# DonghuiZhuo/kube-batch-1

Measured on AMD Instinct MI355X. Metric: pod placements/sec + p50 session latency, 100k nodes × 1M pods, higher is better.
Workload: dtype int64

## Files before the change

kube-batch-1_amd/csrc/engine/engine_placer.h:

```cpp
#pragma once
#include <hip/hip_runtime.h>

#define KBHIP_STAMPS_OFF
#include "../kbhip_batch.h"
#include "../kbhip_engine.h"
#include "engine_dev.h"

namespace kbhip {

static_assert(sizeof(Row) == 4 * (kPkFlags - kPkRow), "the package carries a Row as 28 32-bit words");
static_assert(kEngDescClass + sizeof(TaskClass) / 4 <= kEngDescWords, "a descriptor carries its class");

template <typename ET>
__device__ __forceinline__ Row eng_row_after(const TaskClass& c, const PlaceDec<ET>& D, const Row& base) {
    const int cc = D.cc > 0 ? D.cc : 0;
    const int na = cc < D.ap_l ? cc : D.ap_l;
    return apply_commits(base, c, na, cc - na);
}
template <typename ET>
__device__ __forceinline__ void eng_fit_vals(const Conf& cf, const NodeCols& nc, const DevTables& t,
                                             const TaskClass& c, const PopArgs& a, const PlaceDec<ET>& D,
                                             const Row& base, const int32_t* fit_in, uint32_t fit_raw, uint64_t* g0,
                                             uint64_t* g1) {
    uint32_t fb_base = 0, fb_post = 0;
// ... 191 lines not shown
                                             const TaskClass& c, int node, const Row& r) {
    const uint64_t pw[4] = {0, 0, 0, 0};
    int32_t sc;
    bool passed;
    const int32_t na = cf.score_mult ? na_weight(c, t, nc, node) : 0;
    const uint64_t k1 = dyn_key(cf, c, t, nc, apply_commits(r, c, 1, 0), pw, node, true, na, &sc, &passed);
    return k1 ? key_score(k1) : INT32_MIN;
}
__device__ __forceinline__ bool front_wait(const EngPlacerLds& L, const int* seq, int want) {
    while (__hip_atomic_load(seq, __ATOMIC_RELAXED, __HIP_MEMORY_SCOPE_WORKGROUP) != want) {
        if (!__hip_atomic_load(&L.ok, __ATOMIC_RELAXED, __HIP_MEMORY_SCOPE_WORKGROUP)) return false;
        __builtin_amdgcn_s_sleep(1);
    }
    return true;
}

template <bool LIST>
__device__ __forceinline__ void eng_front_eval(const Conf& cf, const NodeCols& nc, const DevTables& t,
                                               const EngArgs& A, EngPlacerLds& L, uint32_t q, uint32_t dw, int set,
                                               int role) {
    const int lane = eng_lane();
    uint32_t w[8];
#pragma unroll
    for (int i = 0; i < 8; ++i) w[i] = (uint32_t)__builtin_amdgcn_readlane((int)dw, i);
    const EngDesc d = eng_decode(w);
    const PopArgs a = eng_args(d);
    const TaskClass c = eng_class_x(dw);
    const int ring = (int)((q + 3 - set) % 4);
    const int sl = 64 * ring + lane;
    if (!LIST && set == 0) {
        if (!front_wait(L, &L.rows_seq, (int)(q - 1))) return;
        const int node = L.xn[ring][lane];
        if (role == 0) {
            ETL(A, q - 1, 32);
            FrontKey k{0u, 0u, 0u, 0, INT32_MIN};
            if (node >= 0) k = front_key(cf, nc, t, c, a, node, L.rc.row[sl], L.flags[sl]);
            ETL(A, q - 1, 33);
            L.fe[0][lane] = k.e;
            L.ffb[0][lane] = (uint8_t)k.fb;
            L.fkind[0][lane] = (uint8_t)k.kind;
            L.fna[0][lane] = k.na;
            if (k.kind == 2) L.fs1p[0][lane] = k.s1p;
            ETL(A, q - 1, 34);
            L.e[0][lane] = wave_sort_desc(node >= 0 ? k.e : 0u);
            L.fbp[0][lane] = node >= 0 ? (uint8_t)k.fb : (uint8_t)0;
            __builtin_amdgcn_s_waitcnt(0xc07f);
            if (lane == 0) __hip_atomic_store(&L.sort_seq[0], (int)q, __ATOMIC_RELAXED, __HIP_MEMORY_SCOPE_WORKGROUP);
            ETL(A, q - 1, 35);
        } else if (node >= 0) {
            L.fs1a[0][lane] = front_s1a(cf, nc, t, c, node, L.rc.row[sl]);
        }
        return;
    }
    if (set == 0) {
        if (!front_wait(L, &L.xn_seq, (int)(q - 1))) return;
        const int node = L.xn[ring][lane];
        const int src = node >= 0 ? L.srcslot[lane] : 0;
        const bool own_ring = src >= 64 * ring && src < 64 * ring + 64;
        if (role == 0) {
            FrontKey k{0u, 0u, 0u, 0, INT32_MIN};
            if (node >= 0) k = front_key(cf, nc, t, c, a, node, L.rc.row[src], L.flags[src]);
            if (!front_wait(L, &L.rows_seq, (int)(q - 1))) return;
            ETL(A, q - 1, 32);
            const int m = L.ccm[lane];
            if (m == 1 && node >= 0 && !own_ring) {
                if (!front_wait(L, &L.v1_seq[0], (int)q)) return;
                k.e = L.v1e[lane]; k.fb = L.v1fb[lane]; k.kind = L.v1kind[lane]; k.s1p = L.v1s1p[lane];
            }
            const bool slow = node >= 0 && (m > 1 || own_ring);
            if (__ballot(slow) != 0 && slow) k = front_key(cf, nc, t, c, a, node, L.rc.row[sl], L.flags[sl]);
            ETL(A, q - 1, 33);
            L.fe[0][lane] = k.e;
            L.ffb[0][lane] = (uint8_t)k.fb;
            L.fkind[0][lane] = (uint8_t)k.kind;
            L.fna[0][lane] = k.na;
            if (k.kind == 2) L.fs1p[0][lane] = k.s1p;
            ETL(A, q - 1, 34);
            L.e[0][lane] = wave_sort_desc(node >= 0 ? k.e : 0u);
            L.fbp[0][lane] = node >= 0 ? (uint8_t)k.fb : (uint8_t)0;
            __builtin_amdgcn_s_waitcnt(0xc07f);
            if (lane == 0) __hip_atomic_store(&L.sort_seq[0], (int)q, __ATOMIC_RELAXED, __HIP_MEMORY_SCOPE_WORKGROUP);
            ETL(A, q - 1, 35);
        } else {
            int32_t s1 = INT32_MIN;
            if (node >= 0) s1 = front_s1a(cf, nc, t, c, node, L.rc.row[src]);
            if (!front_wait(L, &L.rows_seq, (int)(q - 1))) return;
            const int m = L.ccm[lane];
            if (m == 1 && node >= 0 && !own_ring) {
                if (!front_wait(L, &L.v1_seq[1], (int)q)) return;
                s1 = L.v1s1a[lane];
            }
            const bool slow = node >= 0 && (m > 1 || own_ring);
            if (__ballot(slow) != 0 && slow) s1 = front_s1a(cf, nc, t, c, node, L.rc.row[sl]);
            if (node >= 0) L.fs1a[0][lane] = s1;
        }
        return;
    }
    if (role == 0) ETL(A, q - 1, 32 + 4 * set);
    const int node = L.xn[ring][lane];
    if (role == 0) {
        FrontKey k{0u, 0u, 0u, 0, INT32_MIN};
        if (node >= 0) k = front_key(cf, nc, t, c, a, node, L.rc.row[sl], L.flags[sl]);
        ETL(A, q - 1, 33 + 4 * set);
        L.fe[set][lane] = k.e;
        L.ffb[set][lane] = (uint8_t)k.fb;
        L.fkind[set][lane] = (uint8_t)k.kind;
        L.fna[set][lane] = k.na;
        if (k.kind == 2) L.fs1p[set][lane] = k.s1p;
        bool hashed = false;
        for (int i = 0; i < 4096 && !hashed; ++i) {
            hashed = __hip_atomic_load(&L.hash_seq, __ATOMIC_RELAXED, __HIP_MEMORY_SCOPE_WORKGROUP) == (int)q;
            if (!hashed) __builtin_amdgcn_s_sleep(1);
        }
        ETL(A, q - 1, 34 + 4 * set);
        if (hashed) {
            const bool use = node >= 0 && (set == 1 ? L.x2use[lane] : L.x3use[lane]);
            L.e[set][lane] = wave_sort_desc(use ? k.e : 0u);
            L.fbp[set][lane] = use ? (uint8_t)k.fb : (uint8_t)0;
            __builtin_amdgcn_s_waitcnt(0xc07f);
            if (lane == 0) __hip_atomic_store(&L.sort_seq[set], (int)q, __ATOMIC_RELAXED, __HIP_MEMORY_SCOPE_WORKGROUP);
            ETL(A, q - 1, 35 + 4 * set);
        }
    } else if (node >= 0) {
        L.fs1a[set][lane] = front_s1a(cf, nc, t, c, node, L.rc.row[sl]);
    }
}

__device__ __forceinline__ void eng_front_v1(const Conf& cf, const NodeCols& nc, const DevTables& t,
                                             EngPlacerLds& L, uint32_t q, uint32_t dw, int role) {
    const int lane = eng_lane();
    uint32_t w[8];
#pragma unroll
    for (int i = 0; i < 8; ++i) w[i] = (uint32_t)__builtin_amdgcn_readlane((int)dw, i);
    const PopArgs a = eng_args(eng_decode(w));
    const TaskClass c = eng_class_x(dw);
    if (!front_wait(L, &L.xn_seq, (int)(q - 1))) return;
    const TaskClass& cp = *(const TaskClass*)&L.desc[(q - 1) % 2][kEngDescClass];
    const int ring = (int)((q + 3) % 4);
    const int node = L.xn[ring][lane];
    if (node >= 0) {
        const int src = L.srcslot[lane];
        const Row r = apply_commits(L.rc.row[src], cp, 1, 0);
        if (role == 0) {
            const FrontKey k = front_key(cf, nc, t, c, a, node, r, L.flags[src]);
            L.v1e[lane] = k.e; L.v1fb[lane] = (uint8_t)k.fb; L.v1kind[lane] = (uint8_t)k.kind; L.v1s1p[lane] = k.s1p;
        } else {
            L.v1s1a[lane] = front_s1a(cf, nc, t, c, node, r);
        }
    }
    __builtin_amdgcn_s_waitcnt(0xc07f);
    if (lane == 0) __hip_atomic_store(&L.v1_seq[role], (int)q, __ATOMIC_RELAXED, __HIP_MEMORY_SCOPE_WORKGROUP);
}

template <int K>
__device__ __forceinline__ void front_pkg_store(EngPlacerLds& L, const uint64_t (&v)[16], int base, uint32_t q,
                                                int lane) {
    EngRowCache& rc = L.rc;
#pragma unroll
    for (int i = 0; i < 16; ++i) {
        constexpr int kF0 = 8 * K;
        const int f = kF0 + (i >> 1), e = lane + 64 * (i & 1), sl = base + e;
        const uint32_t x = (uint32_t)v[i];
        if (f == kPkKey) L.pkey[q % 2][e] = x;
        else if (f < kPkFlags) ((uint32_t*)&rc.row[sl])[f - kPkRow] = x;
        else if (f == kPkFlags) L.flags[sl] = (uint8_t)x;
        else if (f == kPkNa) rc.na[sl] = (int32_t)x;
        else rc.s1[sl] = (int32_t)x;
    }
}

template <bool LIST>
__device__ __forceinline__ void eng_front(const Conf& cf, const NodeCols& nc, const DevTables& t, const EngArgs& A,
                                          EngPlacerLds& L, uint32_t q, int wave) {
    const int lane = threadIdx.x & 63;
    EngCtl* ctl = A.ctl;
    EngRowCache& rc = L.rc;
    if (wave == 0) return;
    const int k = wave == 3 ? 0 : wave == 4 ? 1 : wave - 4;
    const EngPkg* pk = A.pkg + (q % kEngSlots);
    uint64_t v[16];
    uint32_t dw;
    if (__hip_atomic_load(&L.ndesc_seq, __ATOMIC_RELAXED, __HIP_MEMORY_SCOPE_WORKGROUP) == (int)q) {
        dw = L.ndesc[lane];
    } else {
        const uint64_t* src = &ctl->desc[q % kEngRing][lane];
        EngWait wt(ctl, kEngDescTicks);
        uint64_t x = 0;
        for (;;) {
            x = ld_sc1(src);
            if (__ballot((uint32_t)(x >> 32) != q) == 0) break;
            if (!wt.tick(kEngErrDesc)) {
                if (wave == 3 && lane == 0) L.ok = 0;
                return;
            }
        }
        dw = (uint32_t)x;
    }
    if (wave == 3) L.desc[q % 2][lane] = dw;
    if (((uint32_t)__builtin_amdgcn_readlane((int)dw, kDwFlags) >> 12 & 0xf) != kEngOpPop) return;
    if (wave == 2) {
        const int r1 = (int)((q + 3) % 4), r2 = (int)((q + 2) % 4), r3 = (int)((q + 1) % 4);
        while (__hip_atomic_load(&L.xn_seq, __ATOMIC_RELAXED, __HIP_MEMORY_SCOPE_WORKGROUP) != (int)(q - 1)) {
            if (!__hip_atomic_load(&L.ok, __ATOMIC_RELAXED, __HIP_MEMORY_SCOPE_WORKGROUP)) return;
            __builtin_amdgcn_s_sleep(1);
        }
        for (int h = lane; h < EngRowCache::kHashN; h += 64) rc.hkey[h] = -1;
        __builtin_amdgcn_s_waitcnt(0xc07f);
        __builtin_amdgcn_wave_barrier();
        const int n1 = L.xn[r1][lane];
        if (n1 >= 0) rc_insert(&rc, n1, 64 * r1 + lane);
        __builtin_amdgcn_s_waitcnt(0xc07f);
        __builtin_amdgcn_wave_barrier();
        const int n2 = L.xn[r2][lane];
        const bool use2 = n2 >= 0 && rc_find(&rc, n2) < 0;
        L.x2use[lane] = use2;
        if (use2) rc_insert(&rc, n2, 64 * r2 + lane);
        if (!LIST) {
            __builtin_amdgcn_s_waitcnt(0xc07f);
            __builtin_amdgcn_wave_barrier();
            const int n3 = L.xn[r3][lane];
            const bool use3 = n3 >= 0 && rc_find(&rc, n3) < 0;
            L.x3use[lane] = use3;
            if (use3) rc_insert(&rc, n3, 64 * r3 + lane);
        }
        __builtin_amdgcn_s_waitcnt(0xc07f);
        if (lane == 0) __hip_atomic_store(&L.hash_seq, (int)q, __ATOMIC_RELAXED, __HIP_MEMORY_SCOPE_WORKGROUP);
        ETL(A, q - 1, 63);
        eng_front_eval<LIST>(cf, nc, t, A, L, q, dw, 0, 1);
        return;
    }
    if constexpr (LIST) {
        if (wave == 1) { eng_front_eval<LIST>(cf, nc, t, A, L, q, dw, 0, 0); return; }
        if (wave == 5) { eng_front_v1(cf, nc, t, L, q, dw, 1); return; }
        if (wave == 3) eng_front_eval<LIST>(cf, nc, t, A, L, q, dw, 1, 1);
        else if (wave == 6) eng_front_eval<LIST>(cf, nc, t, A, L, q, dw, 1, 0);
        else if (wave == 7) eng_front_v1(cf, nc, t, L, q, dw, 0);
    } else {
        if (wave == 1) { eng_front_eval<LIST>(cf, nc, t, A, L, q, dw, 0, 0); return; }
        if (wave == 5) { eng_front_eval<LIST>(cf, nc, t, A, L, q, dw, 1, 1); return; }
        if (wave == 3) eng_front_eval<LIST>(cf, nc, t, A, L, q, dw, 2, 1);
        else if (wave == 6) eng_front_eval<LIST>(cf, nc, t, A, L, q, dw, 1, 0);
        else if (wave == 7) eng_front_eval<LIST>(cf, nc, t, A, L, q, dw, 2, 0);
    }
    ETL(A, q - 1, 56 + k);
    bool got = false;
    if (!eng_poll_tag(ctl, &ctl->pkg_ready[q % kEngSlots][0], q, kEngWaitTicks)) {
        if (k == 0 && lane == 0) L.ok = 0;
        return;
    }
#pragma unroll
    for (int i = 0; i < 16; ++i) v[i] = ld_sc1(&pk->w[8 * k + (i >> 1)][lane + 64 * (i & 1)]);
    EngWait wt(ctl, kEngWaitTicks);
    for (;;) {
        bool miss = false;
#pragma unroll
        for (int i = 0; i < 16; ++i) miss |= (uint32_t)(v[i] >> 32) != q;
        if (__ballot(miss) == 0) { got = true; break; }
#pragma unroll
        for (int i = 0; i < 16; ++i)
            if ((uint32_t)(v[i] >> 32) != q) v[i] = ld_sc1(&pk->w[8 * k + (i >> 1)][lane + 64 * (i & 1)]);
        if (!wt.tick()) break;
    }
    if (got) {
        ETL(A, q - 1, 48 + k);
        const int base = kEngStage + kEngPkgN * (int)(q % 2);
        switch (k) {
            case 0: front_pkg_store<0>(L, v, base, q, lane); break;
            case 1: front_pkg_store<1>(L, v, base, q, lane); break;
            case 2: front_pkg_store<2>(L, v, base, q, lane); break;
            default: front_pkg_store<3>(L, v, base, q, lane); break;
        }
        ETL(A, q - 1, 52 + k);
        if (k == 0) {
            for (int w = 0; w < 4; ++w) { rc.pw[base + lane][w] = 0; rc.pw[base + 64 + lane][w] = 0; }
            bool hashed = false;
            for (int i = 0; i < 4096 && !hashed; ++i) {
                hashed = __hip_atomic_load(&L.hash_seq, __ATOMIC_RELAXED, __HIP_MEMORY_SCOPE_WORKGROUP) == (int)q;
                if (!hashed) __builtin_amdgcn_s_sleep(1);
            }
            ETL(A, q - 1, 62);
            if (hashed) {
                uint32_t w8[8];
#pragma unroll
                for (int i = 0; i < 8; ++i) w8[i] = (uint32_t)__builtin_amdgcn_readlane((int)dw, i);
                eng_drop_stale(L, eng_args(eng_decode(w8)), q);
                __builtin_amdgcn_s_waitcnt(0xc07f);
                if (lane == 0) __hip_atomic_store(&L.drop_seq, (int)q, __ATOMIC_RELAXED, __HIP_MEMORY_SCOPE_WORKGROUP);
                ETL(A, q - 1, 60);
                bool both = false;
                for (int i = 0; i < 4096 && !both; ++i) {
                    both = __hip_atomic_load(&L.sort_seq[1], __ATOMIC_RELAXED, __HIP_MEMORY_SCOPE_WORKGROUP) == (int)q &&
                           (LIST ||
                            __hip_atomic_load(&L.sort_seq[2], __ATOMIC_RELAXED, __HIP_MEMORY_SCOPE_WORKGROUP) == (int)q);
                    if (!both) __builtin_amdgcn_s_sleep(1);
                }
                if (both) {
                    uint32_t top = wave_merge_desc(L.s64[lane], L.e[1][lane]);
                    L.pre64[lane] = LIST ? top : wave_merge_desc(top, L.e[2][lane]);
                    __builtin_amdgcn_s_waitcnt(0xc07f);
                    if (lane == 0) __hip_atomic_store(&L.pre_seq, (int)q, __ATOMIC_RELAXED, __HIP_MEMORY_SCOPE_WORKGROUP);
                    ETL(A, q - 1, 61);
                }
            }
        }
    } else if (k == 0 && lane == 0) {
        L.ok = 0;
    }
}

template <bool LIST>
__device__ __forceinline__ void eng_placer(const Conf& cf, const NodeCols& nc, const DevTables& t, const EngArgs& A,
                                           EngPlacerLds& L) {
    const int lane = threadIdx.x & 63, wave = threadIdx.x >> 6;
    EngCtl* ctl = A.ctl;
    EngRowCache& rc = L.rc;
    for (int i = threadIdx.x; i < 4 * 64; i += kPopThreads) L.xn[i >> 6][i & 63] = -1;
    if (threadIdx.x == 0) {
        L.ok = 1; L.gran_seq = 0; L.ndesc_seq = 0; L.rows_seq = (int)A.first - 1;
        L.hash_seq = L.drop_seq = (int)A.first - 1;
        L.xn_seq = (int)A.first - 1;
        L.v1_seq[0] = L.v1_seq[1] = L.pre_seq = (int)A.first - 1;
        L.sort_seq[0] = L.sort_seq[1] = L.sort_seq[2] = (int)A.first - 1;
        L.apmin = A.first - 1;
    }
    __syncthreads();
    eng_front<LIST>(cf, nc, t, A, L, A.first, wave);
    uint32_t pend = 0;
    for (uint32_t p = A.first;; ++p) {
        const int r1 = (int)((p + 3) % 4), r2 = (int)((p + 2) % 4), r3 = (int)((p + 1) % 4), r0 = (int)(p % 4);
        __syncthreads();
        if (!L.ok) return;
        const EngDesc d = eng_decode(L.desc[p % 2]);
        if (d.op != kEngOpPop) {
            if (wave == 0) eng_publish_done(ctl, &pend);
            return;
        }
        const PopArgs a = eng_args(d);
        const TaskClass& c = *(const TaskClass*)&L.desc[p % 2][kEngDescClass];
        if (wave == 0) {
            ETL(A, p, 0);
            if (lane == 0 && A.tl) A.tl[(size_t)(p % kEngTlSlots) * kEngTlEvents + 31] = p;
        }
        if (wave == 0) {
            if (__hip_atomic_load(&L.drop_seq, __ATOMIC_RELAXED, __HIP_MEMORY_SCOPE_WORKGROUP) != (int)p)
                eng_drop_stale(L, a, p);
            ETL(A, p, 1);
        } else if (wave == 4) {
            const uint64_t x = ld_sc1(&ctl->desc[(p + 1) % kEngRing][lane]);
            if (__ballot((uint32_t)(x >> 32) != p + 1) == 0) {
                L.ndesc[lane] = (uint32_t)x;
                __builtin_amdgcn_s_waitcnt(0xc07f);
                if (lane == 0) __hip_atomic_store(&L.ndesc_seq, (int)(p + 1), __ATOMIC_RELAXED, __HIP_MEMORY_SCOPE_WORKGROUP);
            }
        } else if (wave == 1 || wave == 5 || (!LIST && wave == 6)) {
            const int set = wave == 1 ? 0 : wave - 4;
            const int ring = set == 0 ? r1 : set == 1 ? r2 : r3;
            const int node = L.xn[ring][lane];
            const bool use = node >= 0 && (set == 0 || (set == 1 ? L.x2use[lane] : L.x3use[lane]));
            if (wave == 1) ETL(A, p, 2);
            if (__hip_atomic_load(&L.sort_seq[set], __ATOMIC_RELAXED, __HIP_MEMORY_SCOPE_WORKGROUP) != (int)p) {
                L.e[set][lane] = wave_sort_desc(use ? L.fe[set][lane] : 0u);
                L.fbp[set][lane] = use ? L.ffb[set][lane] : (uint8_t)0;
            }
            if (wave == 1) ETL(A, p, 9);
            if (use) {
                const int sl = 64 * ring + lane;
                const int kind = L.fkind[set][lane];
                rc.na[sl] = L.fna[set][lane];
                rc.s1[sl] = kind == 0 ? INT32_MIN : kind == 2 ? L.fs1p[set][lane] : L.fs1a[set][lane];
            }
        }
        __syncthreads();
        if (wave == 0) ETL(A, p, 3);
        if (wave == 0) {
            uint32_t top;
            if (__hip_atomic_load(&L.pre_seq, __ATOMIC_RELAXED, __HIP_MEMORY_SCOPE_WORKGROUP) == (int)p) {
                top = wave_merge_desc(L.pre64[lane], L.e[0][lane]);
            } else {
                top = wave_merge_desc(L.s64[lane], L.e[0][lane]);
                top = wave_merge_desc(top, L.e[1][lane]);
                if (!LIST) top = wave_merge_desc(top, L.e[2][lane]);
            }
            const uint32_t fbp = (uint32_t)L.fbp[0][lane] | ((uint32_t)L.fbp[1][lane] << 4) |
                                 (LIST ? 0u : ((uint32_t)L.fbp[2][lane] << 8));
#pragma unroll
            for (int q = 0; q < 4; ++q) {
                const int k = __popcll(__ballot((fbp >> q) & 1u)) + __popcll(__ballot((fbp >> (q + 4)) & 1u)) +
                              __popcll(__ballot((fbp >> (q + 8)) & 1u));
                if (lane == q) L.fitin[q] = k;
            }
            const int n = top ? key_node(top, a) : -1;
            ETL(A, p, 44);
            eng_publish_done(ctl, &pend);
            ETL(A, p, 45);
            if constexpr (LIST) {
                if ((int32_t)(L.apmin - (p - kEngLog)) < 0 && !eng_own_apmin(A, L, p - kEngLog)) {
                    if (lane == 0) __hip_atomic_store(&L.ok, 0, __ATOMIC_RELAXED, __HIP_MEMORY_SCOPE_WORKGROUP);
                }
                st_sc1(&ctl->tlog[p % kEngLog][lane], ((uint64_t)p << 32) | (uint32_t)n);
                if (lane == 0) st_sc1(&ctl->tcls[p % kEngLog], ((uint64_t)p << 32) | (uint32_t)a.cls);
            } else {
#pragma unroll
                for (int cp = 0; cp < kEngCandCopies; ++cp)
                    st_sc1(&ctl->cands[p % kEngSlots][cp][lane], ((uint64_t)p << 32) | (uint32_t)n);
            }
            ETL(A, p, 46);
            int src = n >= 0 ? rc_find(&rc, n) : -1;
            if (n >= 0 && src < 0) {
                src = 64 * r0 + lane;
                const Row r = load_row_sc1(nc, n);
                const int32_t na = cf.score_mult ? na_weight(c, t, nc, n) : 0;
                const uint64_t pw[4] = {0, 0, 0, 0};
                rc.row[src] = r;
                L.flags[src] = nc.flags[n];
                rc.na[src] = na;
                rc.s1[src] = depth1_score(cf, nc, t, c, r, pw, n, na, key64_of(top, a));
                for (int w = 0; w < 4; ++w) rc.pw[src][w] = 0;
            }
            L.srcslot[lane] = src;
            L.xn[r0][lane] = n;
            L.wl64[0][lane] = key64_of(top, a);
            __builtin_amdgcn_s_waitcnt(0xc07f);
            if (lane == 0) __hip_atomic_store(&L.xn_seq, (int)p, __ATOMIC_RELAXED, __HIP_MEMORY_SCOPE_WORKGROUP);
            ETL(A, p, 4);
            ETL(A, p, 5);
        }
        if (wave == 0) {
            PlaceDec<uint32_t> D;
            if (place_decide_wave<uint32_t, true>(cf, nc, t, c, a, L.wl64[0], p, &rc, L.srcslot, !A.quick, D)) {
                ETL(A, p, 6);
                if (lane == 0 && A.tl)
                    A.tl[(size_t)(p % kEngTlSlots) * kEngTlEvents + 30] = (uint64_t)D.done | ((uint64_t)D.stop << 8);
                eng_finish<LIST>(cf, nc, t, c, a, A, L, p, r0, D, &pend);
            } else if (lane == 0) {
                __hip_atomic_store(&ctl->err, (uint32_t)kEngErrClass, __ATOMIC_RELAXED, __HIP_MEMORY_SCOPE_AGENT);
                __hip_atomic_store(&L.ok, 0, __ATOMIC_RELAXED, __HIP_MEMORY_SCOPE_WORKGROUP);
            }
        } else {
            if (wave == 5) eng_host_out(A, L, p, d.slot);
            eng_front<LIST>(cf, nc, t, A, L, p + 1, wave);
            if (wave == 3) ETL(A, p, 15);
            if (wave == 1) ETL(A, p, 19);
            if (wave == 5) ETL(A, p, 29);
            if (wave == 7) ETL(A, p, 16);
            if (wave == 6) ETL(A, p, 17);
            if (wave == 4) ETL(A, p, 14);
            if (wave == 2) ETL(A, p, 23);
        }
    }
}

__device__ __forceinline__ void eng_dispatch(const EngArgs& A) {
    const int lane = threadIdx.x & 63;
    EngCtl* ctl = A.ctl;
    uint32_t s = A.first;
    bool idle = false;
    for (;; ++s) {
// ... 64 lines not shown
```

kube-batch-1_amd/csrc/engine/engine_sweep.h:

```cpp
#pragma once
#include <hip/hip_runtime.h>

#define KBHIP_STAMPS_OFF
#include "../kbhip_batch.h"
#include "../kbhip_engine.h"
#include "engine_dev.h"

namespace kbhip {

__device__ __forceinline__ void eng_fit_drop(EngWorkerLds& L, int set, int node, int lo, int cnt) {
    const int lane = threadIdx.x & 63;
    const int o = node - lo;
    const bool own = node >= 0 && o >= 0 && o < cnt;
    uint32_t fb = 0;
    if (own) {
        fb = L.fb[set][o];
        L.fb[set][o] = 0;
    }
#pragma unroll
    for (int q = 0; q < 4; ++q) {
        const int k = __popcll(__ballot((fb >> q) & 1u));
        if (lane == q && k) atomicSub(&L.fitb[set][q], (uint32_t)k);
    }
    __builtin_amdgcn_s_waitcnt(0xc07f);
// ... 178 lines not shown
            for (int q = 0; q < kQ; ++q) {
                if (__ballot((uint32_t)(v0[q] >> 32) != p || (uint32_t)(v1[q] >> 32) != p) == 0) continue;
                v0[q] = ld_sc1(&s[q][lane]);
                v1[q] = ld_sc1(&s[q][64 + lane]);
            }
            if (!wt.tick()) { ok = false; break; }
        }
        if (ok)
#pragma unroll
            for (int q = 0; q < kQ; ++q) wave_merge128_desc(*a0, *a1, (uint32_t)v0[q], (uint32_t)v1[q]);
    }
    return ok;
}

__device__ __forceinline__ bool eng_group_counts(const EngArgs& A, int g, int cg, uint32_t q, bool block, bool* ok) {
    const int lane = threadIdx.x & 63;
    EngCtl* ctl = A.ctl;
    const uint64_t* src0 = A.blists + (size_t)(q % kEngSlots) * A.nw * kEngListWords;
    uint32_t t0 = 0, t1 = 0, t2 = 0, t3 = 0;
    for (int i0 = 0; i0 < cg; i0 += 64) {
        const int i = i0 + lane;
        const uint64_t* s = i < cg ? src0 + (size_t)(g + i * A.ng) * kEngListWords + 128 : nullptr;
        uint64_t x0 = s ? ld_sc1(&s[0]) : ((uint64_t)q << 32), x1 = s ? ld_sc1(&s[1]) : ((uint64_t)q << 32);
        EngWait wt(ctl, kEngWaitTicks);
        while (__ballot((uint32_t)(x0 >> 32) != q || (uint32_t)(x1 >> 32) != q) != 0) {
            if (!block) return false;
            if (!wt.tick()) { *ok = false; return false; }
            if (s) { x0 = ld_sc1(&s[0]); x1 = ld_sc1(&s[1]); }
        }
        const uint32_t y0 = (uint32_t)x0, y1 = (uint32_t)x1;
        t0 += wave_sum_u32(y0 & 0xffff);
        t1 += wave_sum_u32(y0 >> 16);
        t2 += wave_sum_u32(y1 & 0xffff);
        t3 += wave_sum_u32(y1 >> 16);
    }
    uint64_t* dst = A.glists + ((size_t)(q % kEngSlots) * A.ng + g) * kEngListWords;
    if (lane < 4) st_sc1(&dst[128 + lane], ((uint64_t)q << 32) | (lane == 0 ? t0 : lane == 1 ? t1 : lane == 2 ? t2 : t3));
    return true;
}

__device__ __forceinline__ void eng_merger(const EngArgs& A, EngMergerLds& L, int g) {
    const int lane = threadIdx.x & 63, wave = threadIdx.x >> 6;
    EngCtl* ctl = A.ctl;
    const int cg = (A.nw - g + A.ng - 1) / A.ng;
    if (threadIdx.x == 0) L.ok = 1;
    uint32_t cpub = A.first - 1;
    for (uint32_t p = A.first;; ++p) {
        __syncthreads();
        if (!L.ok) return;
        if (wave == 0) {
            bool ok = true;
            const uint64_t* src = &ctl->desc[p % kEngRing][lane];
            EngWait wt(ctl, kEngDescTicks);
            for (;;) {
                const uint64_t x = ld_sc1(src);
                if (__ballot((uint32_t)(x >> 32) != p) == 0) {
                    L.desc[lane] = (uint32_t)x;
                    break;
                }
                if (cpub + 1 < p && eng_group_counts(A, g, cg, p - 1, false, &ok)) cpub = p - 1;
                if (!wt.tick(kEngErrDesc)) { ok = false; break; }
            }
            if (ok && eng_decode(L.desc).op != kEngOpPop && cpub + 1 < p) {
                eng_group_counts(A, g, cg, p - 1, true, &ok);
                cpub = p - 1;
            }
            if (lane == 0) L.ok = ok;
            if (g == 0) ETL(A, p, 24);
        }
        __syncthreads();
        if (!L.ok) return;
        if (eng_decode(L.desc).op != kEngOpPop) return;
        const uint64_t* src0 = A.blists + (size_t)(p % kEngSlots) * A.nw * kEngListWords;
        uint32_t a0 = 0, a1 = 0;
        bool ok = eng_merge_lists(ctl, src0, g, A.ng, cg, p, &a0, &a1);
        if (!ok) L.ok = 0;
        if (g == 0 && wave == 0) ETL(A, p, 25);
        block_merge128_all(L.wl, L.wl2, a0, a1, wave, lane);
        if (!L.ok) return;
        if (wave == 0) {
            uint64_t* dst = A.glists + ((size_t)(p % kEngSlots) * A.ng + g) * kEngListWords;
            st_sc1(&dst[lane], ((uint64_t)p << 32) | L.wl[0][lane]);
            st_sc1(&dst[64 + lane], ((uint64_t)p << 32) | L.wl2[0][lane]);
            if (g == 0) ETL(A, p, 26);
            if (cpub + 1 < p) {
                eng_group_counts(A, g, cg, p - 1, true, &ok);
                cpub = p - 1;
            }
            if (!ok && lane == 0) L.ok = 0;
            if (g == 0) ETL(A, p, 27);
        }
    }
}

__device__ __forceinline__ void eng_final(const Conf& cf, const NodeCols& nc, const DevTables& t, const EngArgs& A,
                          EngMergerLds& L) {
    const int lane = threadIdx.x & 63, wave = threadIdx.x >> 6;
    EngCtl* ctl = A.ctl;
    if (threadIdx.x == 0) L.ok = 1;
    for (uint32_t p = A.first;; ++p) {
        __syncthreads();
        if (!L.ok) return;
        if (wave == 0) {
            const bool ok = eng_wait_desc(ctl, p, L.desc);
            if (lane == 0) L.ok = ok;
            ETL(A, p, 20);
        }
        __syncthreads();
        if (!L.ok) return;
        const EngDesc d = eng_decode(L.desc);
        if (d.op != kEngOpPop) return;
        const PopArgs a = eng_args(d);
        const TaskClass c = eng_class(L.desc);
        uint32_t a0 = 0, a1 = 0;
        bool ok = true;
        if (A.ng == 0) {
            ok = eng_merge_lists(ctl, A.blists + (size_t)(p % kEngSlots) * A.nw * kEngListWords, 0, 1, A.nw, p, &a0,
                                 &a1);
        } else if (wave < A.ng) {
            constexpr int kFinalDepth = 4;
            const uint64_t* s = A.glists + ((size_t)(p % kEngSlots) * A.ng + wave) * kEngListWords;
            uint64_t v0[kFinalDepth], v1[kFinalDepth];
#pragma unroll
            for (int i = 0; i < kFinalDepth; ++i) {
                v0[i] = ld_sc1(&s[lane]);
                v1[i] = ld_sc1(&s[64 + lane]);
                __builtin_amdgcn_s_sleep(2);
            }
            bool got = false;
            EngWait wt(ctl, kEngWaitTicks);
            while (!got) {
#pragma unroll
                for (int i = 0; i < kFinalDepth; ++i) {
                    if (__ballot((uint32_t)(v0[i] >> 32) != p || (uint32_t)(v1[i] >> 32) != p) == 0) {
                        a0 = (uint32_t)v0[i];
                        a1 = (uint32_t)v1[i];
                        got = true;
                        break;
                    }
                    v0[i] = ld_sc1(&s[lane]);
                    v1[i] = ld_sc1(&s[64 + lane]);
                    if (!wt.tick()) break;
                }
                if (!got && ld_sc1(&ctl->err) != 0) break;
            }
            ok = got;
        }
        if (!ok) L.ok = 0;
        block_merge128_all(L.wl, L.wl2, a0, a1, wave, lane);
        if (!L.ok) return;
        if (wave == 0) ETL(A, p, 21);
        EngPkg* pk = A.pkg + (p % kEngSlots);
        const uint64_t tag = (uint64_t)p << 32;
        if (wave < 2) {
            const int e = 64 * wave + lane;
            const uint32_t k = wave == 0 ? L.wl[0][lane] : L.wl2[0][lane];
            const int n = k ? key_node(k, a) : -1;
            uint32_t v[kEngPkgFields];
#pragma unroll
            for (int f = 0; f < kEngPkgFields; ++f) v[f] = 0;
            v[kPkKey] = k;
            if (n >= 0) {
                const Row r = load_row_sc1(nc, n);
                const uint8_t fl = nc.flags[n];
                const int32_t na = cf.score_mult ? na_weight(c, t, nc, n) : 0;
                const uint64_t pw[4] = {0, 0, 0, 0};
                const uint32_t* rw = (const uint32_t*)&r;
#pragma unroll
                for (int f = 0; f < (int)(sizeof(Row) / 4); ++f) v[kPkRow + f] = rw[f];
                v[kPkFlags] = fl;
                v[kPkNa] = (uint32_t)na;
                v[kPkS1] = (uint32_t)depth1_score(cf, nc, t, c, r, pw, n, na, key64_of(k, a));
            }
#pragma unroll
            for (int f = 0; f < kEngPkgFields; ++f) st_sc1(&pk->w[f][e], tag | v[f]);
            asm volatile("s_waitcnt vmcnt(0)" ::: "memory");
        }
        if (wave == 0) ETL(A, p, 22);
        __syncthreads();
        if (threadIdx.x == 0) st_sc1(&ctl->pkg_ready[p % kEngSlots][0], tag | 1u);
    }
}

}
```

kube-batch-1_amd/csrc/kbhip_engine.h:

```cpp
#pragma once
#include <stdint.h>

namespace kbhip {

constexpr int kEngRing = 8;
constexpr int kEngHostRing = 16;
constexpr int kEngSlots = 4;
constexpr int kEngMaxGroups = 8;
constexpr int kEngListWords = 136;
constexpr int kEngMaxNpb = 8192;
constexpr int kEngWorkersMax = 512;
#ifndef KBHIP_CAND_COPIES
#define KBHIP_CAND_COPIES 8
#endif
constexpr int kEngCandCopies = KBHIP_CAND_COPIES;

constexpr int kEngPkgN = 128, kEngPkgFields = 32;
enum : int { kPkKey = 0, kPkRow = 1, kPkFlags = 29, kPkNa = 30, kPkS1 = 31 };
struct EngPkg {
    uint64_t w[kEngPkgFields][kEngPkgN];
};

constexpr int kEngDescWords = 64, kEngDescClass = 8;
enum : int { kDwCls = 0, kDwFlags, kDwMinAvail, kDwReady, kDwEpochSlot, kDwKbase, kDwKshift, kDwKidxmax };
enum : uint32_t { kEngOpPop = 0, kEngOpExit = 1 };

constexpr int kEngLog = 64;
constexpr int kEngOwnMax = 256;
constexpr int kOwnSeg = 1792, kOwnSegs = 64, kOwnMaxN = kOwnSeg * kOwnSegs;
static_assert(kOwnSeg % 256 == 0, "a segment is whole scan steps (64 lanes x 4 nodes)");
constexpr int kOwnLv = 128;

struct EngCtl {
    uint32_t done;
    uint32_t pad0[31];
    uint32_t err;
    uint32_t pad1[31];
    uint32_t arrive;
    uint32_t pad2[63];
    uint64_t desc[kEngRing][kEngDescWords];
    uint64_t cands[kEngSlots][kEngCandCopies][64];
    uint64_t pkg_ready[kEngSlots][16];
    uint64_t tlog[kEngLog][64];
    uint64_t tcls[kEngLog];
    uint32_t own_ap[kEngOwnMax];
};
enum : uint32_t { kEngErrWait = 1, kEngErrDesc = 2, kEngErrClass = 3, kEngErrResident = 4 };

struct EngArgs {
    EngCtl* ctl;
    uint64_t* blists;
    uint64_t* glists;
    EngPkg* pkg;
    const uint64_t* hring;
    uint64_t* hexit;
    uint32_t idle_ticks;
    void* out;
    uint32_t first;
    int nw, npb, ng;
    uint64_t* tl;
    int quick;
    int nown;
    const int32_t* own_cls;
    const int32_t* own_kbase;
    uint8_t* own_fb;
    int kshift, kidxmax;
};
constexpr uint32_t kEngIdleTicks = 10000000u;
constexpr int kEngTlSlots = 32768, kEngTlEvents = 64;

}
```

profiles/engine_tl.py:

```python
#!/usr/bin/env python3
import argparse
import json
import os
import sys

import numpy as np

ROOT = os.path.dirname(os.path.dirname(os.path.abspath(__file__)))
sys.path.insert(0, os.path.join(ROOT, "kube-batch-1_amd"))
import kbgen
import kbhip

SLOTS, EV = 32768, 64


def main():
    ap = argparse.ArgumentParser()
    ap.add_argument("--nodes", type=int, default=100_000)
    ap.add_argument("--pending", type=int, default=800_000)
    ap.add_argument("--workers", type=int, default=0)
    ap.add_argument("--groups", type=int, default=-1)
    ap.add_argument("--out", default="")
    a = ap.parse_args()
    path = f"/tmp/kbhip_bench/c4_{a.nodes}_{a.pending}_{kbgen.BASE_SEED + 4}.kbs"
    if not os.path.exists(path):
        os.makedirs(os.path.dirname(path), exist_ok=True)
        kbgen.gen_c4(path, n_nodes=a.nodes, n_pending=a.pending)
    buf = open(path, "rb").read()
    with kbhip.Session(buf) as s:
        s.allocate()
    with kbhip.Session(buf) as s:
        s.set_option("engine_workers", a.workers)
        s.set_option("engine_groups", a.groups)
        s.set_option("engine_timeline", 1)
        s.allocate()
        st = s.stats()
        raw = np.zeros(SLOTS * EV, np.uint64)
        n = kbhip.lib().kbhip_debug_table(s._h, b"engine_tl", raw.ctypes.data, raw.nbytes)
        assert n == raw.nbytes
    t = raw.reshape(SLOTS, EV).astype(np.int64)
    pops = t[:, 31]
    order = np.argsort(pops)
    t = t[order]
    pops = pops[order]
    keep = (pops > 100) & np.all(t[:, [0, 1, 2, 3, 4, 5, 6, 7, 8, 9, 10, 11, 12, 13, 15, 28]] > 0, axis=1)
    t = t[keep]
    pops = t[:, 31]
    cont = np.diff(pops) == 1
    us = lambda x: float(np.median(x)) / 100.0
    res = {"pops": int(len(t)), "workers": a.workers, "groups": a.groups, "all_stats": {k: (v if isinstance(v, (int, float)) else str(v)) for k, v in st.items()}, "stats": {k: st[k] for k in ("engine_pops", "engine_launches", "engine_workers",
                                                             "alloc_device_s", "batched_pops", "host_wait_s")}}
    per = {}
    per["period"] = us(np.diff(t[:, 0])[cont])
    per["placer 0->3 drop+patch"] = us(t[:, 3] - t[:, 0])
    per["placer 3->4 final list + rows"] = us(t[:, 4] - t[:, 3])
    per["placer 4->5 barrier"] = us(t[:, 5] - t[:, 4])
    per["placer 5->6 decided"] = us(t[:, 6] - t[:, 5])
    per["placer 6->7 rows written"] = us(t[:, 7] - t[:, 6])
    per["placer 6->8 granules (wave 5)"] = us(t[:, 8] - t[:, 6])
    per["placer 5->15 front of next (wave 3, package)"] = us(t[:, 15] - t[:, 5])
    for ev, name in ((19, "wave 1 (pop p-1 cands key)"), (29, "wave 5 (host out + eval)"), (16, "wave 7 (eval + package)"),
                     (17, "wave 6 (eval + package)"), (14, "wave 4 (eval + package)"), (23, "wave 2 (hash)")):
        ok = t[:, ev] > 0
        if ok.any():
            per[f"placer 5->{ev} front {name}"] = us((t[:, ev] - t[:, 5])[ok])
    per["P2 wave0 drop (0->1)"] = us(t[:, 1] - t[:, 0])
    per["P2 wave1 start (0->2)"] = us(t[:, 2] - t[:, 0])
    per["P2 wave1 sort (2->9)"] = us(t[:, 9] - t[:, 2])
    per["placer 7 -> next 0"] = us((t[1:, 0] - t[:-1, 7])[cont])
    fin = np.all(t[:, [20, 21, 22]] > 0, axis=1)
    if fin.any():
        per["final: package flag (22) - placer start (0)"] = us((t[:, 22] - t[:, 0])[fin])
        per["final: desc(20)->merged(21)"] = us((t[:, 21] - t[:, 20])[fin])
        per["final: merged(21)->flag(22)"] = us((t[:, 22] - t[:, 21])[fin])
        f29 = fin & (t[:, 29] > 0)
        if f29.any():
            per["final: merged(21)->cands p-2 seen(29)"] = us((t[:, 29] - t[:, 21])[f29])
            per["final: cands p-2 seen(29,p) - placer P3(4,p-2)"] = us(
                (t[2:, 29] - t[:-2, 4])[((pops[2:] - pops[:-2]) == 2) & f29[2:]])
    lw = t[:, 18] > 0
    if lw.any():
        per["last worker published (18) - worker0 published (13)"] = us((t[:, 18] - t[:, 13])[lw])
        per["last worker published (18) - placer start (0)"] = us((t[:, 18] - t[:, 0])[lw])
    mg = np.all(t[:, [24, 25, 26]] > 0, axis=1)
    if mg.any():
        per["merger0 published (26) - placer start (0)"] = us((t[:, 26] - t[:, 0])[mg])
        per["merger0 lists in (25) - placer start (0)"] = us((t[:, 25] - t[:, 0])[mg])
        per["merger0 desc(24)->lists in(25)"] = us((t[:, 25] - t[:, 24])[mg])
        per["merger0 lists in(25)->pub(26)"] = us((t[:, 26] - t[:, 25])[mg])
        per["merger0 pub(26)->counts(27)"] = us((t[:, 27] - t[:, 26])[mg])
    per["worker0 published (13) - placer start (0)"] = us(t[:, 13] - t[:, 0])
    per["worker0 desc(10)->done(11)"] = us(t[:, 11] - t[:, 10])
    per["worker0 done(11)->eval(12)"] = us(t[:, 12] - t[:, 11])
    per["worker0 eval(12)->pub(13)"] = us(t[:, 13] - t[:, 12])
    per["worker0 pub(13) -> next desc(10)"] = us((t[1:, 10] - t[:-1, 13])[cont])
    per["worker0 published (13, p) - placer P3 (4, p-2)"] = us((t[2:, 13] - t[:-2, 4])[(pops[2:] - pops[:-2]) == 2])
    per["dispatch(28) - placer start(0)"] = us(t[:, 28] - t[:, 0])
    res["median_us"] = {k: round(v, 3) for k, v in per.items()}
    stop = (t[:, 30] >> 8) & 0xff
    res["stop_hist"] = {int(k): int(v) for k, v in zip(*np.unique(stop, return_counts=True))}
    t0all = t[:, 0]
    span = (t0all[-1] - t0all[0]) / 100.0
    dif = np.diff(t0all) / 100.0
    big = np.argsort(dif)[-12:][::-1]
    res["session"] = {"pops_seen": int(len(t0all)), "span_us": round(span, 1), "mean_us": round(span / max(1, len(t0all) - 1), 3),
                      "largest_gaps": [(int(pops[i]), round(float(dif[i]), 1)) for i in big],
                      "gaps_over_20us_total": round(float(dif[dif > 20].sum()), 1), "n_over_20": int((dif > 20).sum())}
    per_all = np.diff(t[:, 0])[cont] / 100.0
    res["period_us"] = {"mean": round(float(per_all.mean()), 3),
                        "quantiles_10_50_90_99": [round(float(np.quantile(per_all, q)), 2) for q in (0.1, 0.5, 0.9, 0.99)],
                        "gaps_over_20us": int((per_all > 20).sum()), "gap_time_over_20us": round(float(per_all[per_all > 20].sum()), 1)}
    dec = (t[:, 6] - t[:, 5]) / 100.0
    res["decide_us_quantiles"] = [round(float(np.quantile(dec, q)), 2) for q in (0.1, 0.25, 0.5, 0.75, 0.9, 0.99)]
    print(json.dumps(res))
    if a.out:
        with open(a.out, "w") as f:
            json.dump(res, f, indent=1)


if __name__ == "__main__":
    main()
```

Baseline: 3.065 million.

## Publish package keys early with separate flag so front cuts list before rows arrive

The sweep's wave 2 now writes the package key field and sets a separate key_ready flag before waves 0/1 compute and publish the row fields. In the non-LIST placer front, wave 3 waits only for the key flag and proceeds to the list cut and merge. Waves 4/6/7 redistribute the row loading across batches off the critical path. The aim is to shorten the dependency chain from package publish to the next placement, at the cost of an extra flag, an extra global store pass, and more polling traffic.

```diff
diff --git a/kube-batch-1_amd/csrc/engine/engine_placer.h b/kube-batch-1_amd/csrc/engine/engine_placer.h
--- a/kube-batch-1_amd/csrc/engine/engine_placer.h
+++ b/kube-batch-1_amd/csrc/engine/engine_placer.h
@@ -367,14 +367,30 @@
     if (lane == 0) __hip_atomic_store(&L.v1_seq[role], (int)q, __ATOMIC_RELAXED, __HIP_MEMORY_SCOPE_WORKGROUP);
 }
 
-template <int K>
-__device__ __forceinline__ void front_pkg_store(EngPlacerLds& L, const uint64_t (&v)[16], int base, uint32_t q,
+template <int F0, int NF>
+__device__ __forceinline__ bool front_pkg_load(EngCtl* ctl, const EngPkg* pk, uint32_t q, int lane,
+                                               uint64_t (&v)[2 * NF]) {
+#pragma unroll
+    for (int i = 0; i < 2 * NF; ++i) v[i] = ld_sc1(&pk->w[F0 + (i >> 1)][lane + 64 * (i & 1)]);
+    EngWait wt(ctl, kEngWaitTicks);
+    for (;;) {
+        bool miss = false;
+#pragma unroll
+        for (int i = 0; i < 2 * NF; ++i) miss |= (uint32_t)(v[i] >> 32) != q;
+        if (__ballot(miss) == 0) return true;
+#pragma unroll
+        for (int i = 0; i < 2 * NF; ++i)
+            if ((uint32_t)(v[i] >> 32) != q) v[i] = ld_sc1(&pk->w[F0 + (i >> 1)][lane + 64 * (i & 1)]);
+        if (!wt.tick()) return false;
+    }
+}
+template <int F0, int NF>
+__device__ __forceinline__ void front_pkg_store(EngPlacerLds& L, const uint64_t (&v)[2 * NF], int base, uint32_t q,
                                                 int lane) {
     EngRowCache& rc = L.rc;
 #pragma unroll
-    for (int i = 0; i < 16; ++i) {
-        constexpr int kF0 = 8 * K;
-        const int f = kF0 + (i >> 1), e = lane + 64 * (i & 1), sl = base + e;
+    for (int i = 0; i < 2 * NF; ++i) {
+        const int f = F0 + (i >> 1), e = lane + 64 * (i & 1), sl = base + e;
         const uint32_t x = (uint32_t)v[i];
         if (f == kPkKey) L.pkey[q % 2][e] = x;
         else if (f < kPkFlags) ((uint32_t*)&rc.row[sl])[f - kPkRow] = x;
@@ -382,6 +398,66 @@
         else if (f == kPkNa) rc.na[sl] = (int32_t)x;
         else rc.s1[sl] = (int32_t)x;
     }
+}
+
+template <bool LIST>
+__device__ __forceinline__ void eng_front_cut(const EngArgs& A, EngPlacerLds& L, uint32_t q, uint32_t dw) {
+    const int lane = threadIdx.x & 63;
+    EngRowCache& rc = L.rc;
+    const int base = kEngStage + kEngPkgN * (int)(q % 2);
+    for (int w = 0; w < 4; ++w) { rc.pw[base + lane][w] = 0; rc.pw[base + 64 + lane][w] = 0; }
+    bool hashed = false;
+    for (int i = 0; i < 4096 && !hashed; ++i) {
+        hashed = __hip_atomic_load(&L.hash_seq, __ATOMIC_RELAXED, __HIP_MEMORY_SCOPE_WORKGROUP) == (int)q;
+        if (!hashed) __builtin_amdgcn_s_sleep(1);
+    }
+    ETL(A, q - 1, 62);
+    if (!hashed) return;
+    uint32_t w8[8];
+#pragma unroll
+    for (int i = 0; i < 8; ++i) w8[i] = (uint32_t)__builtin_amdgcn_readlane((int)dw, i);
+    eng_drop_stale(L, eng_args(eng_decode(w8)), q);
+    __builtin_amdgcn_s_waitcnt(0xc07f);
+    if (lane == 0) __hip_atomic_store(&L.drop_seq, (int)q, __ATOMIC_RELAXED, __HIP_MEMORY_SCOPE_WORKGROUP);
+    ETL(A, q - 1, 60);
+    bool both = false;
+    for (int i = 0; i < 4096 && !both; ++i) {
+        both = __hip_atomic_load(&L.sort_seq[1], __ATOMIC_RELAXED, __HIP_MEMORY_SCOPE_WORKGROUP) == (int)q &&
+               (LIST || __hip_atomic_load(&L.sort_seq[2], __ATOMIC_RELAXED, __HIP_MEMORY_SCOPE_WORKGROUP) == (int)q);
+        if (!both) __builtin_amdgcn_s_sleep(1);
+    }
+    if (both) {
+        uint32_t top = wave_merge_desc(L.s64[lane], L.e[1][lane]);
+        L.pre64[lane] = LIST ? top : wave_merge_desc(top, L.e[2][lane]);
+        __builtin_amdgcn_s_waitcnt(0xc07f);
+        if (lane == 0) __hip_atomic_store(&L.pre_seq, (int)q, __ATOMIC_RELAXED, __HIP_MEMORY_SCOPE_WORKGROUP);
+        ETL(A, q - 1, 61);
+    }
+}
+
+template <int B>
+__device__ __forceinline__ bool front_rows_batch(EngCtl* ctl, EngPlacerLds& L, const EngPkg* pk, uint32_t p,
+                                                 int lane) {
+    constexpr int kF0 = kPkRow + 8 * B, kNF = kF0 + 8 <= kEngPkgFields ? 8 : kEngPkgFields - kF0;
+    uint64_t v[2 * kNF];
+    if (!front_pkg_load<kF0, kNF>(ctl, pk, p, lane, v)) return false;
+    front_pkg_store<kF0, kNF>(L, v, kEngStage + kEngPkgN * (int)(p % 2), p, lane);
+    return true;
+}
+template <int B0, int NB>
+__device__ __forceinline__ bool eng_front_rows(const EngArgs& A, EngPlacerLds& L, uint32_t q) {
+    const int lane = threadIdx.x & 63;
+    EngCtl* ctl = A.ctl;
+    const EngPkg* pk = A.pkg + (q % kEngSlots);
+    if (!eng_poll_tag(ctl, &ctl->pkg_ready[q % kEngSlots][0], q, kEngWaitTicks)) return false;
+    if (B0 == 0) ETL(A, q, 49);
+    if (!front_rows_batch<B0>(ctl, L, pk, q, lane)) return false;
+    if (B0 == 0) ETL(A, q, 50);
+    if constexpr (NB > 1) {
+        if (!front_rows_batch<B0 + 1>(ctl, L, pk, q, lane)) return false;
+    }
+    ETL(A, q, B0 == 0 ? 53 : B0 == 2 ? 54 : 55);
+    return true;
 }
 
 template <bool LIST>
@@ -393,7 +469,6 @@
     if (wave == 0) return;
     const int k = wave == 3 ? 0 : wave == 4 ? 1 : wave - 4;
     const EngPkg* pk = A.pkg + (q % kEngSlots);
-    uint64_t v[16];
     uint32_t dw;
     if (__hip_atomic_load(&L.ndesc_seq, __ATOMIC_RELAXED, __HIP_MEMORY_SCOPE_WORKGROUP) == (int)q) {
         dw = L.ndesc[lane];
@@ -457,67 +532,52 @@
         else if (wave == 6) eng_front_eval<LIST>(cf, nc, t, A, L, q, dw, 1, 0);
         else if (wave == 7) eng_front_eval<LIST>(cf, nc, t, A, L, q, dw, 2, 0);
     }
+    if constexpr (!LIST) {
+        if (wave != 3) {
+            const bool ok = wave == 4   ? eng_front_rows<0, 2>(A, L, q)
+                            : wave == 6 ? eng_front_rows<2, 1>(A, L, q)
+                                        : eng_front_rows<3, 1>(A, L, q);
+            if (!ok && lane == 0) __hip_atomic_store(&L.ok, 0, __ATOMIC_RELAXED, __HIP_MEMORY_SCOPE_WORKGROUP);
+            return;
+        }
+        ETL(A, q - 1, 56);
+        uint64_t kv[2];
+        bool ok = eng_poll_tag(ctl, &ctl->key_ready[q % kEngSlots][0], q, kEngWaitTicks);
+        ETL(A, q - 1, 48);
+        ok = ok && front_pkg_load<kPkKey, 1>(ctl, pk, q, lane, kv);
+        if (!ok) {
+            if (lane == 0) L.ok = 0;
+            return;
+        }
+        front_pkg_store<kPkKey, 1>(L, kv, 0, q, lane);
+        ETL(A, q - 1, 52);
+        eng_front_cut<LIST>(A, L, q, dw);
+        return;
+    }
     ETL(A, q - 1, 56 + k);
-    bool got = false;
     if (!eng_poll_tag(ctl, &ctl->pkg_ready[q % kEngSlots][0], q, kEngWaitTicks)) {
         if (k == 0 && lane == 0) L.ok = 0;
         return;
     }
-#pragma unroll
-    for (int i = 0; i < 16; ++i) v[i] = ld_sc1(&pk->w[8 * k + (i >> 1)][lane + 64 * (i & 1)]);
-    EngWait wt(ctl, kEngWaitTicks);
-    for (;;) {
-        bool miss = false;
-#pragma unroll
-        for (int i = 0; i < 16; ++i) miss |= (uint32_t)(v[i] >> 32) != q;
-        if (__ballot(miss) == 0) { got = true; break; }
-#pragma unroll
-        for (int i = 0; i < 16; ++i)
-            if ((uint32_t)(v[i] >> 32) != q) v[i] = ld_sc1(&pk->w[8 * k + (i >> 1)][lane + 64 * (i & 1)]);
-        if (!wt.tick()) break;
+    uint64_t v[16];
+    const int base = kEngStage + kEngPkgN * (int)(q % 2);
+    bool got;
+    switch (k) {
+        case 0: got = front_pkg_load<0, 8>(ctl, pk, q, lane, v); break;
+        case 1: got = front_pkg_load<8, 8>(ctl, pk, q, lane, v); break;
+        case 2: got = front_pkg_load<16, 8>(ctl, pk, q, lane, v); break;
+        default: got = front_pkg_load<24, 8>(ctl, pk, q, lane, v); break;
     }
     if (got) {
         ETL(A, q - 1, 48 + k);
-        const int base = kEngStage + kEngPkgN * (int)(q % 2);
         switch (k) {
-            case 0: front_pkg_store<0>(L, v, base, q, lane); break;
-            case 1: front_pkg_store<1>(L, v, base, q, lane); break;
-            case 2: front_pkg_store<2>(L, v, base, q, lane); break;
-            default: front_pkg_store<3>(L, v, base, q, lane); break;
+            case 0: front_pkg_store<0, 8>(L, v, base, q, lane); break;
+            case 1: front_pkg_store<8, 8>(L, v, base, q, lane); break;
+            case 2: front_pkg_store<16, 8>(L, v, base, q, lane); break;
+            default: front_pkg_store<24, 8>(L, v, base, q, lane); break;
         }
         ETL(A, q - 1, 52 + k);
-        if (k == 0) {
-            for (int w = 0; w < 4; ++w) { rc.pw[base + lane][w] = 0; rc.pw[base + 64 + lane][w] = 0; }
-            bool hashed = false;
-            for (int i = 0; i < 4096 && !hashed; ++i) {
-                hashed = __hip_atomic_load(&L.hash_seq, __ATOMIC_RELAXED, __HIP_MEMORY_SCOPE_WORKGROUP) == (int)q;
-                if (!hashed) __builtin_amdgcn_s_sleep(1);
-            }
-            ETL(A, q - 1, 62);
-            if (hashed) {
-                uint32_t w8[8];
-#pragma unroll
-                for (int i = 0; i < 8; ++i) w8[i] = (uint32_t)__builtin_amdgcn_readlane((int)dw, i);
-                eng_drop_stale(L, eng_args(eng_decode(w8)), q);
-                __builtin_amdgcn_s_waitcnt(0xc07f);
-                if (lane == 0) __hip_atomic_store(&L.drop_seq, (int)q, __ATOMIC_RELAXED, __HIP_MEMORY_SCOPE_WORKGROUP);
-                ETL(A, q - 1, 60);
-                bool both = false;
-                for (int i = 0; i < 4096 && !both; ++i) {
-                    both = __hip_atomic_load(&L.sort_seq[1], __ATOMIC_RELAXED, __HIP_MEMORY_SCOPE_WORKGROUP) == (int)q &&
-                           (LIST ||
-                            __hip_atomic_load(&L.sort_seq[2], __ATOMIC_RELAXED, __HIP_MEMORY_SCOPE_WORKGROUP) == (int)q);
-                    if (!both) __builtin_amdgcn_s_sleep(1);
-                }
-                if (both) {
-                    uint32_t top = wave_merge_desc(L.s64[lane], L.e[1][lane]);
-                    L.pre64[lane] = LIST ? top : wave_merge_desc(top, L.e[2][lane]);
-                    __builtin_amdgcn_s_waitcnt(0xc07f);
-                    if (lane == 0) __hip_atomic_store(&L.pre_seq, (int)q, __ATOMIC_RELAXED, __HIP_MEMORY_SCOPE_WORKGROUP);
-                    ETL(A, q - 1, 61);
-                }
-            }
-        }
+        if (k == 0) eng_front_cut<LIST>(A, L, q, dw);
     } else if (k == 0 && lane == 0) {
         L.ok = 0;
     }
diff --git a/kube-batch-1_amd/csrc/engine/engine_sweep.h b/kube-batch-1_amd/csrc/engine/engine_sweep.h
--- a/kube-batch-1_amd/csrc/engine/engine_sweep.h
+++ b/kube-batch-1_amd/csrc/engine/engine_sweep.h
@@ -354,6 +354,13 @@
         if (wave == 0) ETL(A, p, 21);
         EngPkg* pk = A.pkg + (p % kEngSlots);
         const uint64_t tag = (uint64_t)p << 32;
+        if (wave == 2) {
+            st_sc1(&pk->w[kPkKey][lane], tag | L.wl[0][lane]);
+            st_sc1(&pk->w[kPkKey][64 + lane], tag | L.wl2[0][lane]);
+            asm volatile("s_waitcnt vmcnt(0)" ::: "memory");
+            if (lane == 0) st_sc1(&ctl->key_ready[p % kEngSlots][0], tag | 1u);
+            ETL(A, p, 57);
+        }
         if (wave < 2) {
             const int e = 64 * wave + lane;
             const uint32_t k = wave == 0 ? L.wl[0][lane] : L.wl2[0][lane];
@@ -361,7 +368,6 @@
             uint32_t v[kEngPkgFields];
 #pragma unroll
             for (int f = 0; f < kEngPkgFields; ++f) v[f] = 0;
-            v[kPkKey] = k;
             if (n >= 0) {
                 const Row r = load_row_sc1(nc, n);
                 const uint8_t fl = nc.flags[n];
@@ -375,7 +381,7 @@
                 v[kPkS1] = (uint32_t)depth1_score(cf, nc, t, c, r, pw, n, na, key64_of(k, a));
             }
 #pragma unroll
-            for (int f = 0; f < kEngPkgFields; ++f) st_sc1(&pk->w[f][e], tag | v[f]);
+            for (int f = kPkRow; f < kEngPkgFields; ++f) st_sc1(&pk->w[f][e], tag | v[f]);
             asm volatile("s_waitcnt vmcnt(0)" ::: "memory");
         }
         if (wave == 0) ETL(A, p, 22);
diff --git a/kube-batch-1_amd/csrc/kbhip_engine.h b/kube-batch-1_amd/csrc/kbhip_engine.h
--- a/kube-batch-1_amd/csrc/kbhip_engine.h
+++ b/kube-batch-1_amd/csrc/kbhip_engine.h
@@ -41,6 +41,7 @@
     uint64_t desc[kEngRing][kEngDescWords];
     uint64_t cands[kEngSlots][kEngCandCopies][64];
     uint64_t pkg_ready[kEngSlots][16];
+    uint64_t key_ready[kEngSlots][16];
     uint64_t tlog[kEngLog][64];
     uint64_t tcls[kEngLog];
     uint32_t own_ap[kEngOwnMax];
diff --git a/profiles/engine_tl.py b/profiles/engine_tl.py
--- a/profiles/engine_tl.py
+++ b/profiles/engine_tl.py
@@ -64,6 +64,26 @@
         ok = t[:, ev] > 0
         if ok.any():
             per[f"placer 5->{ev} front {name}"] = us((t[:, ev] - t[:, 5])[ok])
+    nxt = np.zeros(len(t), bool)
+    nxt[:-1] = cont
+    for ev, name in ((56, "key wave starts polling"), (48, "key flag seen (single flag: package block in registers)"),
+                     (52, "keys in LDS"), (60, "list cut"), (61, "list merged with sets 1, 2")):
+        ok = nxt & (t[:, ev] > 0)
+        if ok.any():
+            per[f"front of p+1: {name} ({ev}) - P3 publish of p (4)"] = us((t[:, ev] - t[:, 4])[ok])
+            per[f"front of p+1: {name} ({ev}) before next placer start (0)"] = us(
+                (t[1:, 0] - t[:-1, ev])[ok[:-1]])
+    for ev, name in ((49, "rows' flag seen (wave 4)"), (50, "wave 4's first batch in LDS"),
+                     (53, "rows in LDS, wave 4's share"), (54, "rows in LDS, wave 6's share"),
+                     (55, "rows in LDS, wave 7's share")):
+        ok = t[:, ev] > 0
+        if ok.any():
+            per[f"rows of p: {name} ({ev}) - placer start (0)"] = us((t[:, ev] - t[:, 0])[ok])
+    ok = (t[:, 57] > 0) & (t[:, 21] > 0) & (t[:, 22] > 0)
+    if ok.any():
+        per["final: merged(21)->key flag(57)"] = us((t[:, 57] - t[:, 21])[ok])
+        per["final: key flag(57)->package flag(22)"] = us((t[:, 22] - t[:, 57])[ok])
+    per["P3 publish (4) - placer start (0)"] = us(t[:, 4] - t[:, 0])
     per["P2 wave0 drop (0->1)"] = us(t[:, 1] - t[:, 0])
     per["P2 wave1 start (0->2)"] = us(t[:, 2] - t[:, 0])
     per["P2 wave1 sort (2->9)"] = us(t[:, 9] - t[:, 2])
```

Result: slower. 2.936 million (-4.2%).
